# pingpongshow/RIA

Hardware: AMD Instinct MI355X
Metric: frames/s demod+LDPC-decoded, OFDM QAM16 R1/2 1024-FFT (higher is better)
Workload: dtype f32; 1 GPU; OFDM QAM16 R1/2 + LDPC min-sum, Watterson moderate fading 20 dB, 4400000 frames (100000 per step per GPU), full decodeFixedFrame; frame_samples=18432, batch_per_gpu=100000, channel=2

## Files before the change

### ria_amd/csrc/ldpc_fast.hip.h

```cpp
#pragma once
#include <hip/hip_runtime.h>
#include <stdint.h>

#include <type_traits>

#include "../../include/ria_gpu.h"
#include "devmath.h"
#include "ldpc_kernels.hip.h"

namespace ria {

struct ShapeR12 {
    static constexpr int NR = 6, NC = 6;
    static constexpr int kCascadeWaves = 3;
    static constexpr int kCv = 24;
    static constexpr int ne(int r) { constexpr int t[NR] = {6, 6, 5, 4, 2, 1}; return t[r]; }
    static constexpr int nm(int r) { constexpr int t[NR] = {6, 5, 4, 2, 1, 1}; return t[r]; }
    static constexpr int dv(int r) { constexpr int t[NC] = {5, 4, 4, 4, 4, 4}; return t[r]; }
};
struct ShapeR13 {
    static constexpr int NR = 6, NC = 6;
    static constexpr int kCascadeWaves = 3;
    static constexpr int kCv = 24;
    static constexpr int ne(int r) { constexpr int t[NR] = {6, 6, 5, 3, 3, 1}; return t[r]; }
// ... 108 lines not shown
}

template <int OFF>
__device__ __forceinline__ void lds_store_tid(uint32_t base, float v) {
    static_assert(OFF >= 0 && OFF < 65536, "16-bit DS offset");
    if constexpr (!kAddTid) {
        *(lds_float_ptr)(uintptr_t)(base + static_cast<uint32_t>(threadIdx.x) * 4u + OFF) = v;
        return;
    }
    asm volatile("s_mov_b32 m0, %1\n\ts_nop 0\n\tds_write_addtid_b32 %0 offset:%2" : : "v"(v), "s"(base), "n"(OFF) : "memory", "m0");
}
template <int N, int OFF, int STEP>
__device__ __forceinline__ void lds_store_tid_n(uint32_t base, const float (&v)[N]) {
    static_assert(N >= 1 && N <= 6 && OFF >= 0 && OFF + (N - 1) * STEP < 65536, "up to six 16-bit DS offsets");
    if constexpr (!kAddTid) {
#pragma unroll
        for (int i = 0; i < N; ++i) *(lds_float_ptr)(uintptr_t)(base + static_cast<uint32_t>(threadIdx.x) * 4u + OFF + i * STEP) = v[i];
        return;
    }
    if constexpr (N == 1)
        asm volatile("s_mov_b32 m0, %1\n\ts_nop 0\n\tds_write_addtid_b32 %0 offset:%2" : : "v"(v[0]), "s"(base), "n"(OFF) : "memory", "m0");
    else if constexpr (N == 2)
        asm volatile("s_mov_b32 m0, %2\n\ts_nop 0\n\tds_write_addtid_b32 %0 offset:%3\n\tds_write_addtid_b32 %1 offset:%4"
                     : : "v"(v[0]), "v"(v[1]), "s"(base), "n"(OFF), "n"(OFF + STEP) : "memory", "m0");
    else if constexpr (N == 3)
        asm volatile("s_mov_b32 m0, %3\n\ts_nop 0\n\tds_write_addtid_b32 %0 offset:%4\n\tds_write_addtid_b32 %1 offset:%5\n\tds_write_addtid_b32 %2 offset:%6"
                     : : "v"(v[0]), "v"(v[1]), "v"(v[2]), "s"(base), "n"(OFF), "n"(OFF + STEP), "n"(OFF + 2 * STEP) : "memory", "m0");
    else if constexpr (N == 4)
        asm volatile("s_mov_b32 m0, %4\n\ts_nop 0\n\tds_write_addtid_b32 %0 offset:%5\n\tds_write_addtid_b32 %1 offset:%6\n\tds_write_addtid_b32 %2 offset:%7\n\tds_write_addtid_b32 %3 offset:%8"
                     : : "v"(v[0]), "v"(v[1]), "v"(v[2]), "v"(v[3]), "s"(base), "n"(OFF), "n"(OFF + STEP), "n"(OFF + 2 * STEP), "n"(OFF + 3 * STEP) : "memory", "m0");
    else if constexpr (N == 5)
        asm volatile("s_mov_b32 m0, %5\n\ts_nop 0\n\tds_write_addtid_b32 %0 offset:%6\n\tds_write_addtid_b32 %1 offset:%7\n\tds_write_addtid_b32 %2 offset:%8\n\tds_write_addtid_b32 %3 offset:%9\n\tds_write_addtid_b32 %4 offset:%10"
                     : : "v"(v[0]), "v"(v[1]), "v"(v[2]), "v"(v[3]), "v"(v[4]), "s"(base), "n"(OFF), "n"(OFF + STEP), "n"(OFF + 2 * STEP), "n"(OFF + 3 * STEP), "n"(OFF + 4 * STEP) : "memory", "m0");
    else
        asm volatile("s_mov_b32 m0, %6\n\ts_nop 0\n\tds_write_addtid_b32 %0 offset:%7\n\tds_write_addtid_b32 %1 offset:%8\n\tds_write_addtid_b32 %2 offset:%9\n\tds_write_addtid_b32 %3 offset:%10\n\tds_write_addtid_b32 %4 offset:%11\n\tds_write_addtid_b32 %5 offset:%12"
                     : : "v"(v[0]), "v"(v[1]), "v"(v[2]), "v"(v[3]), "v"(v[4]), "v"(v[5]), "s"(base), "n"(OFF), "n"(OFF + STEP), "n"(OFF + 2 * STEP), "n"(OFF + 3 * STEP), "n"(OFF + 4 * STEP), "n"(OFF + 5 * STEP) : "memory", "m0");
}
__device__ __forceinline__ uint32_t med3u(uint32_t a, uint32_t b, uint32_t c) {
    uint32_t d;
    asm("v_med3_u32 %0, %1, %2, %3" : "=v"(d) : "v"(a), "v"(b), "v"(c));
    return d;
}
__device__ __forceinline__ float med3_abs(float x, float b, float c) { return __builtin_amdgcn_fmed3f(__builtin_fabsf(x), b, c); }
__device__ __forceinline__ float min_abs(float x, float b) { return __builtin_fminf(__builtin_fabsf(x), b); }
__device__ __forceinline__ float min3_abs(float a, float b, float c) { return __builtin_fminf(__builtin_fminf(__builtin_fabsf(a), __builtin_fabsf(b)), __builtin_fabsf(c)); }
__device__ __forceinline__ float med3_abs3(float a, float b, float c) { return __builtin_amdgcn_fmed3f(__builtin_fabsf(a), __builtin_fabsf(b), __builtin_fabsf(c)); }
__device__ __forceinline__ float min2_abs(float a, float b) { return __builtin_fminf(__builtin_fabsf(a), __builtin_fabsf(b)); }
__device__ __forceinline__ float max2_abs(float a, float b) { return __builtin_fmaxf(__builtin_fabsf(a), __builtin_fabsf(b)); }
__device__ __forceinline__ float min_raw(float a, float b) { return __builtin_fminf(a, b); }
template <int N>
__device__ __forceinline__ void two_smallest_abs(const float (&w)[N], float& lo, float& mid) {
    static_assert(N >= 2 && N <= 7, "row degree");
    if constexpr (N == 2) { lo = min2_abs(w[0], w[1]); mid = max2_abs(w[0], w[1]); }
    else {
        lo = min3_abs(w[0], w[1], w[2]); mid = med3_abs3(w[0], w[1], w[2]);
        if constexpr (N >= 6) {
            const float l2 = min3_abs(w[3], w[4], w[5]), m2 = med3_abs3(w[3], w[4], w[5]);
            const float x = min_raw(mid, m2);
            mid = __builtin_amdgcn_fmed3f(lo, l2, x);
            lo = min_raw(lo, l2);
            if constexpr (N == 7) { mid = med3_abs(w[6], lo, mid); lo = min_abs(w[6], lo); }
        } else {
            if constexpr (N >= 4) { mid = med3_abs(w[3], lo, mid); lo = min_abs(w[3], lo); }
            if constexpr (N >= 5) { mid = med3_abs(w[4], lo, mid); lo = min_abs(w[4], lo); }
        }
    }
}
__device__ __forceinline__ uint32_t bfi(uint32_t mask, uint32_t a, uint32_t b) { return (mask & a) | (~mask & b); }

__device__ __forceinline__ float llr_canon(float x) {
    x = (x < 1e30f) ? x : 1e30f;
    x = (-1e30f < x) ? x : -1e30f;
    return x + 0.0f;
}

#ifndef RIA_SINGLE_PREFETCH
#define RIA_SINGLE_PREFETCH 2
#endif
template <class S, int NCV = (kCvRegs ? 1024 : S::kCv), int PF = RIA_SINGLE_PREFETCH>
__device__ inline int fast_decode(FastState<S>& st, const FastCode& c, unsigned char* __restrict__ lds,
                                  float factor, int max_iter, int lane, bool* ok) {
    using I = ShapeInfo<S>;
    const uint32_t lane4 = lds_addr(lds) + static_cast<uint32_t>(lane) * 4u;
    const uint32_t kAbs = 0x7fffffffu;
    const uint32_t m0base = lds_addr(lds);
    static_for<0, S::NR>([&](auto R_) __attribute__((always_inline)) {
        constexpr int r = decltype(R_)::value;
#pragma unroll
        for (int s = 0; s < S::ne(r); ++s) {
            const float v0 = 0.0f;
            if (I::row_off(r) + s < NCV) st.cv[I::row_off(r) + s] = v0;
            else lds_sf(lane4 + 256u * (I::row_off(r) + s), v0);
        }
    });
#pragma unroll
    for (int r = 0; r < S::NC; ++r) lds_sf(lane4 + 4u * (I::tot_word + 64 * r), st.li[r]);
    lds_sf(lane4 + 4u * I::zero_word, 0.0f);
    lds_sf(lane4 + 4u * I::big_word, kPadTotal);
#pragma unroll
    for (int r = 0; r < S::NR; ++r) { st.pv[r] = st.lp[r]; st.pt[r] = 0.0f; }
    wave_sync();
    float hi = __builtin_inff();
    int it = 0;
    bool success = false;
    for (; it < max_iter; ++it) {
        uint32_t syn = 0;
        float tt[I::TS];
        auto gather_round = [&](auto G_) __attribute__((always_inline)) {
            constexpr int g = decltype(G_)::value;
            if constexpr (g < S::NR) {
#pragma unroll
                for (int s = 0; s < S::ne(g); ++s) tt[I::row_off(g) + s] = lds_f(st.rv[I::row_off(g) + s]);
            }
        };
        static_for<0, PF>([&](auto G_) __attribute__((always_inline)) { gather_round(G_); });
        static_for<0, S::NR>([&](auto R_) __attribute__((always_inline)) {
            constexpr int r = decltype(R_)::value;
            constexpr int NE = S::ne(r);
            constexpr int off = I::row_off(r);
            gather_round(std::integral_constant<int, r + PF>{});
            float t[NE], cold[NE];
#pragma unroll
            for (int s = 0; s < NE; ++s) {
                t[s] = tt[off + s];
                if (off + s < NCV) cold[s] = st.cv[off + s];
                else cold[s] = lds_f(lane4 + 256u * (off + s));
            }
            const float pvr = st.pv[r];
            uint32_t par = f2u(st.pt[r]);
            uint32_t sgn = f2u(pvr);
            float min1, min2;
            float v[NE + 1];
#pragma unroll
            for (int s = 0; s < NE; ++s) v[s] = t[s] - cold[s];
            v[NE] = pvr;
            two_smallest_abs<NE + 1>(v, min1, min2);
            min1 = min_raw(min1, hi);
            min2 = min_raw(min2, hi);
#pragma unroll
            for (int s = 0; s < NE; s += 2) {
                if (s + 1 < NE) {
                    par = __builtin_amdgcn_bitop3_b32(par, f2u(t[s]), f2u(t[s + 1]), 0x96);
                    sgn = __builtin_amdgcn_bitop3_b32(sgn, f2u(v[s]), f2u(v[s + 1]), 0x96);
                } else {
                    par ^= f2u(t[s]);
                    sgn ^= f2u(v[s]);
                }
            }
            syn |= par;
            const uint32_t dS = bfi(kAbs, f2u(min1) ^ f2u(min2), sgn);
            float o[NE];
#pragma unroll
            for (int s = 0; s < NE; ++s) o[s] = u2f(dS ^ f2u(__builtin_amdgcn_fmed3f(v[s], min2, -min2))) * factor;
            lds_store_tid_n<NE, 256 * off, 256>(m0base, o);
            static_for<0, NE>([&](auto S_) __attribute__((always_inline)) {
                constexpr int s = decltype(S_)::value;
                if constexpr (off + s < NCV) st.cv[off + s] = o[s];
            });
            {
                const float c2v = u2f(dS ^ f2u(__builtin_amdgcn_fmed3f(pvr, min2, -min2))) * factor;
                const float tot = st.lp[r] + c2v;
                st.pv[r] = tot - c2v;
                st.pt[r] = tot;
            }
        });
        if (it > 0 && __ballot(static_cast<int>(syn) < 0) == 0ull) { success = true; --it; break; }
        hi = 50.0f;
        wave_sync();
        constexpr int NCE = []() constexpr { int n = 0; for (int r = 0; r < S::NC; ++r) if (S::dv(r) > 0) n = r + 1; return n; }();
        float totv[NCE > 0 ? NCE : 1];
        static_for<0, NCE>([&](auto R_) __attribute__((always_inline)) {
            constexpr int r = decltype(R_)::value;
            constexpr int DV = S::dv(r);
            constexpr int off = I::col_off(r);
            float cv[DV > 0 ? DV : 1];
#pragma unroll
            for (int d = 0; d < DV; ++d) cv[d] = lds_f(st.cs[off + d]);
            float tot = st.li[r];
#pragma unroll
            for (int d = 0; d < DV; ++d) tot = tot + cv[d];
            totv[r] = tot;
        });
        static_for<0, (NCE + 5) / 6>([&](auto G_) __attribute__((always_inline)) {
            constexpr int g0 = 6 * decltype(G_)::value, gn = (NCE - g0 < 6) ? NCE - g0 : 6;
            float tv[gn];
#pragma unroll
            for (int i = 0; i < gn; ++i) tv[i] = totv[g0 + i];
            lds_store_tid_n<gn, 4 * (I::tot_word + 64 * g0), 256>(m0base, tv);
        });
        wave_sync();
    }
    if (!success) {
        uint32_t syn = 0;
        static_for<0, S::NR>([&](auto R_) __attribute__((always_inline)) {
            constexpr int r = decltype(R_)::value;
            constexpr int off = I::row_off(r);
            uint32_t par = f2u(st.pt[r]);
#pragma unroll
            for (int s = 0; s < S::ne(r); ++s) par ^= f2u(lds_f(st.rv[off + s]));
            syn |= par;
        });
        if (max_iter > 0 && __ballot(static_cast<int>(syn) < 0) == 0ull) { success = true; it = max_iter - 1; }
    }
    *ok = success;
    return success ? it : max_iter;
}

template <class S>
__device__ inline void fast_pack(const FastState<S>& st, const FastCode& c, unsigned char* lds, uint8_t* out, int nbytes,
                                 int lane) {
    using I = ShapeInfo<S>;
    (void)st;
    lane = opaque_lane(lane);
    unsigned long long* masks = reinterpret_cast<unsigned long long*>(lds);
    const int nr = (c.k + 63) / 64;
    for (int r = 0; r < nr; ++r) {
        const int j = lane + 64 * r;
        bool bit = false;
        if (j < c.k) bit = (f2u(lds_f(lds_addr(lds) + 4u * (I::tot_word + c.col_pos[j]))) >> 31) != 0u;
        unsigned long long mk = __ballot(bit);
        if (lane == 0) masks[r] = mk;
    }
    wave_sync();
    for (int b = lane; b < nbytes; b += 64) out[b] = static_cast<uint8_t>(__brev(static_cast<unsigned>(lds[b])) >> 24);
    wave_sync();
}

struct CascadeWin { unsigned int lock; unsigned int iters; uint8_t bytes[72]; };

struct DecodeCtl {
    unsigned int n_entries;
    unsigned int next_unit;
    unsigned int n_list1;
    unsigned int next_z;
    unsigned int queue_fault;
    unsigned int pad_[3];
};
#define RIA_QUEUE_GUARD(guard, total, ctl) \
    if (++(guard) > (total) + 2u) { if (threadIdx.x == 0) atomicExch(&(ctl)->queue_fault, 1u); break; }

constexpr int kNumFactors = 5;
__device__ __constant__ float kFactors[kNumFactors] = {0.9375f, 0.875f, 0.75f, 0.625f, 0.5f};
struct CwResult {
    uint8_t state[kNumFactors];
    uint8_t pad[kNumFactors - 2];
    uint16_t iters[kNumFactors];
};

struct FastDecodeArgs {
    FastCode c;
    const uint16_t* gather;
    const float* llr;
    int llr_stride;
    int n_frames;
    uint32_t flags;
    uint8_t* info_out;
    ria_decode_status* status;
    const uint16_t* crc_bit;
    const uint16_t* crc_init;
    DecodeCtl* ctl;
    unsigned int* entries;
    unsigned int* best;
    unsigned int* list1;
    CwResult* res;
    uint8_t* res_bytes;
    CascadeWin* win;
    float* staged;
    unsigned int* l1idx;
    unsigned int* l1hash;
    uint32_t* seed_ws;
};

constexpr int kStageFloats = 12 * 64;
constexpr int kStageFrameFloats = 2688;

constexpr float kIdleRowLlr = 1e30f;

template <class S>
__device__ inline void fast_gather_llr(FastState<S>& st, const FastCode& c, const float* fl, const uint16_t* gather,
                                       int cw, int lane) {
    lane = opaque_lane(lane);
#pragma unroll
    for (int r = 0; r < S::NC; ++r) {
        const uint32_t j = c.col_at[lane + 64 * r];
        st.li[r] = (j != 0xFFFFu) ? llr_canon(fl[gather[cw * 648 + j]]) : 0.0f;
    }
#pragma unroll
    for (int r = 0; r < S::NR; ++r) {
        const uint32_t i = c.check_at[lane + 64 * r];
        st.lp[r] = (i != 0xFFFFu) ? llr_canon(fl[gather[cw * 648 + c.k + i]]) : kIdleRowLlr;
    }
}

template <class S>
__device__ inline void fast_load_staged(FastState<S>& st, const float* __restrict__ src, int lane) {
    static_assert((S::NC + S::NR) * 64 <= kStageFloats, "stage slot too small");
    lane = opaque_lane(lane);
#pragma unroll
    for (int r = 0; r < S::NC; ++r) st.li[r] = src[r * 64 + lane];
#pragma unroll
    for (int r = 0; r < S::NR; ++r) st.lp[r] = src[(S::NC + r) * 64 + lane];
}

template <class S, int NCV = S::kCv>
__device__ inline void fast_unit(FastState<S>& st, const FastDecodeArgs& A, unsigned char* lds, unsigned fc, int f, int lane,
                                 const float* staged = nullptr) {
    const FastCode& c = A.c;
    if (staged) fast_load_staged(st, staged, lane);
    else fast_gather_llr(st, c, A.llr + static_cast<size_t>(fc >> 2) * A.llr_stride, A.gather, fc & 3, lane);
    bool ok;
    int it = fast_decode<S, NCV>(st, c, lds, kFactors[f], c.max_iter, lane, &ok);
    if (ok) fast_pack(st, c, lds, A.res_bytes + (static_cast<size_t>(fc) * kNumFactors + f) * c.bytes_per_cw,
                      c.bytes_per_cw, lane);
    if (lane == 0) { A.res[fc].state[f] = ok ? 2 : 1; A.res[fc].iters[f] = static_cast<uint16_t>(it); }
}

#ifndef RIA_PRIMARY_NCV
#define RIA_PRIMARY_NCV 0
#endif
template <class S>
__global__ __launch_bounds__(64) void fast_primary_kernel(FastDecodeArgs A) {
    extern __shared__ __attribute__((aligned(16))) unsigned char smem[];
    const int lane = threadIdx.x;
    const unsigned b = blockIdx.x, g = b >> 5, r = b & 31u, cw = r >> 3, x = r & 7u;
    const unsigned frame = 8u * g + x;
    if (frame >= static_cast<unsigned>(A.n_frames)) return;
    FastState<S> st;
    fast_load_tables(st, A.c, smem, lane);
    fast_unit<S, RIA_PRIMARY_NCV>(st, A, smem, 4u * frame + cw, 0, lane);
}

__global__ void fast_mark_kernel(FastDecodeArgs A) {
    int frame = blockIdx.x * blockDim.x + threadIdx.x;
    if (frame >= A.n_frames) return;
    if (!(A.flags & (RIA_DECODE_PHASE0 | RIA_DECODE_PERTURB))) return;
    bool failed = false;
    for (int cw = 0; cw < 4; ++cw) {
        unsigned fc = static_cast<unsigned>(frame) * 4u + cw;
        failed = failed || A.res[fc].state[0] != 2;
        if (failed) {
            const unsigned i = atomicAdd(&A.ctl->n_list1, 1u);
            A.list1[i] = fc;
            A.l1idx[fc] = i;
        }
    }
}

__device__ inline uint32_t fast_hash16(const float* fl, const uint16_t* gather, int cw, int lane) {
    const uint32_t mine = f2u(fl[gather[cw * 648 + (lane & 15)]]);
    uint32_t h = 0;
    for (int j = 0; j < 16; ++j) {
        uint32_t u = __shfl(mine, j);
        h ^= u + 0x9e3779b9u + (h << 6) + (h >> 2);
    }
    return h;
}

template <class S>
__global__ __launch_bounds__(256) void fast_stage_kernel(FastDecodeArgs A) {
    __shared__ float fr[kStageFrameFloats];
    const FastCode& c = A.c;
    const int tid = threadIdx.x, lane = tid & 63, wave = tid >> 6;
    const unsigned n = A.ctl->n_list1;
    const int nfl = A.llr_stride < kStageFrameFloats ? A.llr_stride : kStageFrameFloats;
    for (unsigned i = blockIdx.x; i < n; i += gridDim.x) {
        const unsigned fc = A.list1[i], cw = fc & 3u;
        const float* fl = A.llr + static_cast<size_t>(fc >> 2) * A.llr_stride;
        __syncthreads();
        for (int q = tid; q < nfl; q += 256) fr[q] = fl[q];
        __syncthreads();
        float* dst = A.staged + static_cast<size_t>(i) * kStageFloats;
        for (int r = wave; r < S::NC + S::NR; r += 4) {
            float v;
            if (r < S::NC) {
                const uint32_t j = c.col_at[lane + 64 * r];
                v = (j != 0xFFFFu) ? llr_canon(fr[A.gather[cw * 648 + j]]) : 0.0f;
            } else {
                const uint32_t k = c.check_at[lane + 64 * (r - S::NC)];
                v = (k != 0xFFFFu) ? llr_canon(fr[A.gather[cw * 648 + c.k + k]]) : kIdleRowLlr;
            }
            dst[r * 64 + lane] = v;
        }
        if (wave == 0) {
            const uint32_t h = fast_hash16(fr, A.gather, cw, lane);
            if (lane == 0) A.l1hash[i] = h;
        }
    }
}

template <class S>
__global__ __launch_bounds__(64) void fast_phase0_kernel(FastDecodeArgs A) {
    extern __shared__ __attribute__((aligned(16))) unsigned char smem[];
    const int lane = threadIdx.x;
    const unsigned total = A.ctl->n_list1 * 4u;
    if (blockIdx.x >= total) return;
    FastState<S> st;
    fast_load_tables(st, A.c, smem, lane);
    unsigned guard = 0;
    for (;;) {
        RIA_QUEUE_GUARD(guard, total, A.ctl)
        unsigned u = atomicAdd(&A.ctl->next_z, lane == 0 ? 1u : 0u);
        u = __builtin_amdgcn_readfirstlane(u);
        if (u >= total) break;
        fast_unit<S>(st, A, smem, A.list1[u >> 2], 1 + static_cast<int>(u & 3u), lane, A.staged + static_cast<size_t>(u >> 2) * kStageFloats);
    }
}

__global__ void fast_chain_kernel(FastDecodeArgs A) {
    int frame = blockIdx.x * blockDim.x + threadIdx.x;
    if (frame >= A.n_frames) return;
    const int bpc = A.c.bytes_per_cw;
    int f = 0;
    ria_decode_status* s = A.status + frame;
    for (int cw = 0; cw < 4; ++cw) {
        const unsigned fc = static_cast<unsigned>(frame) * 4u + cw;
        const CwResult r = A.res[fc];
        int accept = -1, attempts = 1, iters = r.iters[f];
        if (r.state[f] == 2) accept = f;
        else {
            if (A.flags & RIA_DECODE_PHASE0) {
                for (int t = 1; t <= 4 && accept < 0; ++t) { attempts++; if (r.state[t] == 2) { accept = t; iters = r.iters[t]; } }
                f = 0;
            }
            if (accept < 0 && (A.flags & RIA_DECODE_PERTURB)) {
                f = 1;
                unsigned e = atomicAdd(&A.ctl->n_entries, 1u);
                A.entries[e] = fc;
                A.best[e] = 0xFFFFFFFFu;
                A.win[e].lock = 0u;
            }
        }
        uint8_t* out = A.info_out + static_cast<size_t>(fc) * bpc;
        if (accept >= 0) {
            const uint8_t* src = A.res_bytes + (static_cast<size_t>(fc) * kNumFactors + accept) * bpc;
            for (int b = 0; b < bpc; ++b) out[b] = src[b];
        } else {
            for (int b = 0; b < bpc; ++b) out[b] = 0;
        }
        s->cw_ok[cw] = accept >= 0 ? 1 : 0;
        s->iterations[cw] = static_cast<uint16_t>(iters);
        s->attempts[cw] = static_cast<uint8_t>(attempts);
    }
}

#ifndef RIA_CASCADE_GROUP
#define RIA_CASCADE_GROUP 4
#endif
constexpr int kCascadeGroup = RIA_CASCADE_GROUP;
constexpr unsigned kCascadeGroups = (kRetryAttempts + kCascadeGroup - 1) / kCascadeGroup;
constexpr size_t kSeedWsWords = static_cast<size_t>(kCascadeGroup) * 624;

template <class S>
__device__ inline float fast_perturb(FastState<S>& st, const FastCode& c, const float* base_i, const float* base_p,
                                     uint32_t* mt, float* normal, const uint32_t* ws, int j, int a, int lane) {
    uint32_t seed; float sigma, factor; int kind;
    lane = opaque_lane(lane);
    retry_transform_params(a, 0u, &seed, &sigma, &factor, &kind);
    const bool noise = sigma != 0.0f;
    if (noise) {
        mt_load_group_state<kCascadeGroup>(mt, ws, j, lane);
        normal648_state(mt, normal, lane);
    }
    auto tf = [&](float v, float nz) {
        if (kind == 1) { v = (v < 10.0f) ? v : 10.0f; v = (-10.0f < v) ? v : -10.0f; }
        else if (kind == 2) v = v * 0.5f;
        else if (kind == 3) { v = (v < 6.0f) ? v : 6.0f; v = (-6.0f < v) ? v : -6.0f; }
        else if (kind == 4) v = (v >= 0.0f) ? 1.0f : -1.0f;
        else if (kind == 5) v = v * 0.25f;
        return v + (nz * sigma + 0.0f);
    };
#pragma unroll
    for (int r = 0; r < S::NC; ++r) {
        const uint32_t q = c.col_at[lane + 64 * r];
        const float nz = (noise && q != 0xFFFFu) ? normal[q] : 0.0f;
        st.li[r] = (q != 0xFFFFu) ? llr_canon(tf(base_i[r], nz)) : 0.0f;
    }
#pragma unroll
    for (int r = 0; r < S::NR; ++r) {
        const uint32_t i = c.check_at[lane + 64 * r];
        const float nz = (noise && i != 0xFFFFu) ? normal[c.k + i] : 0.0f;
        st.lp[r] = (i != 0xFFFFu) ? llr_canon(tf(base_p[r], nz)) : kIdleRowLlr;
    }
    wave_sync();
    return factor;
}

template <class S>
__global__ __launch_bounds__(64) __attribute__((amdgpu_waves_per_eu(S::kCascadeWaves))) void fast_cascade_kernel(FastDecodeArgs A) {
    extern __shared__ __attribute__((aligned(16))) unsigned char smem[];
    const FastCode& c = A.c;
    const int lane = threadIdx.x;
    float* msg = reinterpret_cast<float*>(smem);
    const unsigned int n_entries = A.ctl->n_entries;
    const unsigned int total = n_entries * kCascadeGroups;
    if (total == 0) return;
    FastState<S> st;
    fast_load_tables(st, c, smem, lane);
    unsigned guard = 0;
    for (;;) {
        RIA_QUEUE_GUARD(guard, total, A.ctl)
        unsigned int u = atomicAdd(&A.ctl->next_unit, lane == 0 ? 1u : 0u);
        u = __builtin_amdgcn_readfirstlane(u);
        if (u >= total) break;
        const unsigned int g = u / n_entries, e = u - g * n_entries, a0 = g * kCascadeGroup;
        unsigned int b = __hip_atomic_load(&A.best[e], __ATOMIC_RELAXED, __HIP_MEMORY_SCOPE_AGENT);
        b = __builtin_amdgcn_readfirstlane(b);
        if (b < a0) continue;
        const unsigned int li = A.l1idx[A.entries[e]];
        uint32_t* ws = A.seed_ws + static_cast<size_t>(blockIdx.x) * kSeedWsWords;
        mt_seed_group<kCascadeGroup>(ws, A.l1hash[li], a0, opaque_lane(lane));
#pragma unroll 1
        for (int j = 0; j < kCascadeGroup; ++j) {
            const unsigned int a = a0 + static_cast<unsigned>(j);
            if (a >= kRetryAttempts) break;
            if (j > 0) {
                b = __hip_atomic_load(&A.best[e], __ATOMIC_RELAXED, __HIP_MEMORY_SCOPE_AGENT);
                b = __builtin_amdgcn_readfirstlane(b);
                if (b < a) break;
            }
            fast_load_staged(st, A.staged + static_cast<size_t>(li) * kStageFloats, lane);
            float bi[S::NC], bp[S::NR];
#pragma unroll
            for (int r = 0; r < S::NC; ++r) bi[r] = st.li[r];
#pragma unroll
            for (int r = 0; r < S::NR; ++r) bp[r] = st.lp[r];
            float factor = fast_perturb(st, c, bi, bp, reinterpret_cast<uint32_t*>(msg), msg + 640, ws, j, static_cast<int>(a), lane);
            bool ok;
            const int it = fast_decode<S>(st, c, smem, factor, c.max_iter, lane, &ok);
            if (!ok) continue;
            unsigned int prev = atomicMin(&A.best[e], lane == 0 ? a : 0xFFFFFFFFu);
            prev = __builtin_amdgcn_readfirstlane(prev);
            if (a < prev) {
                CascadeWin* w = A.win + e;
                bool mine = false;
                for (unsigned spin = 0; spin < (1u << 20); ++spin) {
                    unsigned got = atomicCAS(&w->lock, 0u, lane == 0 ? 1u : 0u);
                    got = __builtin_amdgcn_readfirstlane(got);
                    if (got == 0u) { mine = true; break; }
                    __builtin_amdgcn_s_sleep(1);
                }
                if (!mine) { if (lane == 0) atomicExch(&A.ctl->queue_fault, 1u); break; }
                __threadfence();
                unsigned int cur = __hip_atomic_load(&A.best[e], __ATOMIC_RELAXED, __HIP_MEMORY_SCOPE_AGENT);
                cur = __builtin_amdgcn_readfirstlane(cur);
                if (cur == a) {
                    fast_pack(st, c, smem, w->bytes, c.bytes_per_cw, lane);
                    if (lane == 0) w->iters = static_cast<unsigned int>(it);
                }
                __threadfence();
                if (lane == 0) atomicExch(&w->lock, 0u);
            }
            break;
        }
    }
}

__global__ __launch_bounds__(256) void fast_finalize_kernel(FastDecodeArgs A) {
    const unsigned int n_entries = A.ctl->n_entries;
    const int bpc = A.c.bytes_per_cw;
    for (unsigned int e = blockIdx.x * blockDim.x + threadIdx.x; e < n_entries; e += gridDim.x * blockDim.x) {
        const unsigned int fc = A.entries[e], frame = fc >> 2, cw = fc & 3;
        const unsigned int a = A.best[e];
        ria_decode_status* s = A.status + frame;
        if (a >= 34u) { s->attempts[cw] = static_cast<uint8_t>(s->attempts[cw] + 34); continue; }
        const CascadeWin* w = A.win + e;
        uint8_t* out = A.info_out + (static_cast<size_t>(frame) * 4 + cw) * bpc;
        for (int b = 0; b < bpc; ++b) out[b] = w->bytes[b];
        s->cw_ok[cw] = 1;
        s->iterations[cw] = static_cast<uint16_t>(w->iters);
        s->attempts[cw] = static_cast<uint8_t>(s->attempts[cw] + a + 1);
    }
}

__device__ inline bool decode_fault_mark(const DecodeCtl* ctl, ria_decode_status* s, uint8_t* info, int info_bytes, int lane) {
    if (__hip_atomic_load(&ctl->queue_fault, __ATOMIC_RELAXED, __HIP_MEMORY_SCOPE_AGENT) == 0u) return false;
    for (int b = lane; b < info_bytes; b += 64) info[b] = 0;
    if (lane == 0) {
        for (int cw = 0; cw < 4; ++cw) s->cw_ok[cw] = 0;
        s->frame_valid = 0; s->needs_recovery = 0; s->reserved[0] = 0; s->reserved[1] = 0xEE;
    }
    return true;
}
constexpr uint8_t kDecodeFaultMarker = 0xEE;

__global__ __launch_bounds__(256) void frame_validate_kernel(uint8_t* __restrict__ info, int bpc, int n_frames,
                                                             const uint16_t* __restrict__ crc_bit,
                                                             const uint16_t* __restrict__ crc_init,
                                                             ria_decode_status* __restrict__ status, const DecodeCtl* ctl) {
    __shared__ uint8_t flat_all[4][4 * 68];
    const int lane = threadIdx.x & 63, wave = threadIdx.x >> 6;
    const int frame = blockIdx.x * 4 + wave;
    if (frame >= n_frames) return;
    uint8_t* flat = flat_all[wave];
    ria_decode_status* s = status + frame;
    if (decode_fault_mark(ctl, s, info + static_cast<size_t>(frame) * 4 * bpc, 4 * bpc, lane)) return;
    const bool all_ok = s->cw_ok[0] && s->cw_ok[1] && s->cw_ok[2] && s->cw_ok[3];
    int valid = 0, quirk = 0;
    if (all_ok) {
        for (int b = lane; b < 4 * bpc; b += 64) flat[b] = info[static_cast<size_t>(frame) * 4 * bpc + b];
        wave_sync();
        bool magic = flat[0] == 0x55 && flat[1] == 0x4C;
        int t = flat[2];
        bool ctl = (t == 0x10 || t == 0x11 || t == 0x16 || t == 0x17 || t == 0x20 || t == 0x21 || t == 0x15 || t == 0x40);
        int plen = (flat[13] << 8) | flat[14];
        int expected = ctl ? 20 : 17 + plen + 2;
        for (int cw = 1; cw < 4; ++cw) if (cw * bpc < expected && flat[cw * bpc] == 0xD5) quirk = 1;
        if (magic && !quirk) {
            if (ctl) {
                uint32_t crc = crc16_wave(flat, 18, crc_bit, crc_init, lane);
                valid = crc == static_cast<uint32_t>((flat[18] << 8) | flat[19]);
            } else {
                uint32_t hc = crc16_wave(flat, 15, crc_bit, crc_init, lane);
                if (hc == static_cast<uint32_t>((flat[15] << 8) | flat[16]) && expected <= 4 * bpc) {
                    uint32_t fc = crc16_wave(flat, expected - 2, crc_bit, crc_init, lane);
                    valid = fc == static_cast<uint32_t>((flat[expected - 2] << 8) | flat[expected - 1]);
                }
            }
        }
    }
    if (lane == 0) {
        s->frame_valid = static_cast<uint8_t>(valid);
        s->needs_recovery = static_cast<uint8_t>(all_ok && !valid);
        s->reserved[0] = static_cast<uint8_t>(quirk);
        s->reserved[1] = 0;
    }
}

__global__ __launch_bounds__(256) void decode_fault_kernel(const DecodeCtl* ctl, ria_decode_status* __restrict__ status, uint8_t* __restrict__ info,
                                                           int bpc, int n_frames) {
    const int lane = threadIdx.x & 63, frame = blockIdx.x * 4 + (threadIdx.x >> 6);
    if (frame >= n_frames) return;
    (void)decode_fault_mark(ctl, status + frame, info + static_cast<size_t>(frame) * 4 * bpc, 4 * bpc, lane);
}

#ifndef RIA_ROWS_NCV
#define RIA_ROWS_NCV (kCvRegs ? 1024 : S::kCv)
#endif
#ifdef RIA_ROWS_WAVES
#define RIA_ROWS_ATTR __attribute__((amdgpu_waves_per_eu(RIA_ROWS_WAVES, RIA_ROWS_WAVES)))
#else
#define RIA_ROWS_ATTR
#endif
template <class S>
__global__ __launch_bounds__(64) RIA_ROWS_ATTR void fast_rows_kernel(FastCode c, const float* __restrict__ llr, int n_cw, int max_iter,
                                                       float factor, uint8_t* __restrict__ out, uint8_t* __restrict__ ok_out,
                                                       uint16_t* __restrict__ iters_out) {
    extern __shared__ __attribute__((aligned(16))) unsigned char smem[];
    const int lane = threadIdx.x;
    FastState<S> st;
    fast_load_tables(st, c, smem, lane);
    const int nb = (c.k + 7) / 8;
    for (int cw = blockIdx.x; cw < n_cw; cw += gridDim.x) {
        const float* l = llr + static_cast<size_t>(cw) * 648;
        const int ln = opaque_lane(lane);
#pragma unroll
        for (int r = 0; r < S::NC; ++r) { const uint32_t j = c.col_at[ln + 64 * r]; st.li[r] = (j != 0xFFFFu) ? llr_canon(l[j]) : 0.0f; }
#pragma unroll
        for (int r = 0; r < S::NR; ++r) { const uint32_t i = c.check_at[ln + 64 * r]; st.lp[r] = (i != 0xFFFFu) ? llr_canon(l[c.k + i]) : kIdleRowLlr; }
        bool ok;
        int it = fast_decode<S, RIA_ROWS_NCV>(st, c, smem, factor, max_iter, lane, &ok);
        fast_pack(st, c, smem, out + static_cast<size_t>(cw) * nb, nb, lane);
        if (lane == 0) { ok_out[cw] = ok ? 1 : 0; iters_out[cw] = static_cast<uint16_t>(it); }
    }
}

template <class S>
__global__ __launch_bounds__(64) void fast_robust_kernel(FastCode c, const float* __restrict__ llr, int n_cw,
                                                         uint8_t* __restrict__ out, uint8_t* __restrict__ ok_out,
                                                         uint16_t* __restrict__ iters_out, uint8_t* __restrict__ tries_out) {
    extern __shared__ __attribute__((aligned(16))) unsigned char smem[];
    const int lane = threadIdx.x;
    FastState<S> st;
    fast_load_tables(st, c, smem, lane);
    const int nb = (c.k + 7) / 8;
    for (int cw = blockIdx.x; cw < n_cw; cw += gridDim.x) {
        const float* l = llr + static_cast<size_t>(cw) * 648;
#pragma unroll
        for (int r = 0; r < S::NC; ++r) { const uint32_t j = c.col_at[lane + 64 * r]; st.li[r] = (j != 0xFFFFu) ? llr_canon(l[j]) : 0.0f; }
#pragma unroll
        for (int r = 0; r < S::NR; ++r) { const uint32_t i = c.check_at[lane + 64 * r]; st.lp[r] = (i != 0xFFFFu) ? llr_canon(l[c.k + i]) : kIdleRowLlr; }
        bool ok = false;
        int it = 0, tries = 0;
#pragma unroll 1
        for (int f = 0; f < kNumFactors && !ok; ++f) {
            it = fast_decode(st, c, smem, kFactors[f], c.max_iter, lane, &ok);
            ++tries;
        }
        fast_pack(st, c, smem, out + static_cast<size_t>(cw) * nb, nb, lane);
        if (lane == 0) {
            ok_out[cw] = ok ? 1 : 0; iters_out[cw] = static_cast<uint16_t>(it);
            if (tries_out) tries_out[cw] = static_cast<uint8_t>(tries);
        }
    }
}

}
```

### ria_amd/csrc/recovery_kernels.hip.h

```cpp
#pragma once
#include <hip/hip_runtime.h>
#include <stdint.h>

#include "ldpc_fast.hip.h"
#include "sort_exact.hpp"

namespace ria {

struct RecCtx {
    uint8_t* cw;
    uint8_t* fd;
    uint8_t* trial;
    Suspect* sus;
    int* stack;
    uint16_t* sd;
    uint16_t* lists;
    int sus_cap;
    unsigned long long* dbg;
    int bpc;
    const uint16_t* crc_bit;
    const uint16_t* crc_init;
    int lane;
};

// ... 149 lines not shown
    if (lane < fin) mine = v[lane];
    int rank = 0;
    for (int j = 0; j < fin; ++j) {
        const float kj = __builtin_bit_cast(float, __builtin_amdgcn_readlane(__builtin_bit_cast(int, mine.abs_llr), j));
        rank += (kj < mine.abs_llr || (j < lane && !(mine.abs_llr < kj))) ? 1 : 0;
    }
    wave_sync();
    if (lane < fin) v[rank] = mine;
    wave_sync();
}

constexpr int kRecOverflow = 2;
constexpr int kRecSmallCap = 320;
template <class LlrFn>
__device__ inline int rec_search(const RecCtx& x, LlrFn llr) {
    const int bpc = x.bpc, lane = x.lane;
    auto stamp = [&](int k) { if (x.dbg && lane == 0) x.dbg[k] = __builtin_readcyclecounter(); };
    stamp(0);
    const int flen = rec_reassemble(x, x.fd);
    if (flen == 0) {
        const int tb = bpc * 8;
        const uint8_t* c0 = x.cw;
        const uint32_t hsyn = crc16_wave(c0, 15, x.crc_bit, x.crc_init, lane) ^ static_cast<uint32_t>((c0[15] << 8) | c0[16]);
        const uint32_t msyn = static_cast<uint32_t>((c0[0] << 8) | c0[1]) ^ 0x554Cu;
        auto dh = [&](int b) -> uint32_t {
            const int by = b >> 3, bit = b & 7;
            if (by < 15) return x.crc_bit[(14 - by) * 8 + bit];
            if (by == 15) return 1u << (8 + bit);
            if (by == 16) return 1u << bit;
            return 0u;
        };
        auto dm = [&](int b) -> uint32_t {
            const int by = b >> 3, bit = b & 7;
            if (by == 0) return 1u << (8 + bit);
            if (by == 1) return 1u << bit;
            return 0u;
        };
        const uint32_t d0 = (dh(lane) << 16) | dm(lane), d1 = (dh(lane + 64) << 16) | dm(lane + 64), d2 = (dh(lane + 128) << 16) | dm(lane + 128);
        const uint32_t syn2 = (hsyn << 16) | msyn;
        auto d_of = [&](int b) -> uint32_t {
            if (b >= 192) return 0u;
            const uint32_t r = (b < 64) ? d0 : (b < 128) ? d1 : d2;
            return static_cast<uint32_t>(__builtin_amdgcn_readlane(static_cast<int>(r), b & 63));
        };
        auto for_matches = [&](uint32_t want, int from, auto f) -> bool {
            for (int base = 0; base < 192 && base < tb; base += 64) {
                const int b = base + lane;
                const uint32_t dv = (base == 0) ? d0 : (base == 64) ? d1 : d2;
                unsigned long long hits = __ballot(b >= from && b < tb && dv == want);
                while (hits) {
                    const int bb = base + __builtin_ctzll(hits);
                    hits &= hits - 1;
                    if (f(bb)) return true;
                }
            }
            if (want == 0u)
                for (int bb = (from > 192 ? from : 192); bb < tb; ++bb) if (f(bb)) return true;
            return false;
        };
        if (for_matches(syn2, 0, [&](int bb) {
                rec_flip(x, bb >> 3, bb & 7);
                if (rec_try(x)) return true;
                rec_flip(x, bb >> 3, bb & 7);
                return false; })) return true;
        for (int b1 = 0; b1 < tb; ++b1) {
            const uint32_t want = syn2 ^ d_of(b1);
            if (want == 0u) {
                rec_flip(x, b1 >> 3, b1 & 7);
                const int tl = rec_reassemble(x, x.trial);
                bool ctl2 = false; int plen2 = 0;
                const bool hdr = tl > 0 && rec_parse_header(x, x.trial, tl, &ctl2, &plen2);
                const int exp2 = 17 + plen2 + 2;
                bool done = false;
                if (hdr && !ctl2 && tl >= exp2) {
                    const uint32_t s2 = static_cast<uint32_t>((x.trial[exp2 - 2] << 8) | x.trial[exp2 - 1]) ^
                                        crc16_wave(x.trial, exp2 - 2, x.crc_bit, x.crc_init, lane);
                    const int from = (b1 + 1 > 136) ? b1 + 1 : 136;
                    for (int base = (from & ~63); base < tb && !done; base += 64) {
                        const int b2 = base + lane, by = b2 >> 3, bit = b2 & 7;
                        uint32_t dl = 0u;
                        if (b2 < tb) {
                            if (by < exp2 - 2) dl = x.crc_bit[(exp2 - 3 - by) * 8 + bit];
                            else if (by < exp2) dl = 1u << (bit + 8 * (exp2 - 1 - by));
                        }
                        unsigned long long hits = __ballot(b2 >= from && b2 < tb && dl == s2);
                        while (hits && !done) {
                            const int bb = base + __builtin_ctzll(hits);
                            hits &= hits - 1;
                            rec_flip(x, bb >> 3, bb & 7);
                            if (rec_try(x)) done = true; else rec_flip(x, bb >> 3, bb & 7);
                        }
                    }
                } else if (hdr && ctl2) {
                    done = true;
                } else if (!hdr) {
                    for (int bb = (b1 + 1 > 136) ? b1 + 1 : 136; bb < tb && !done; ++bb) {
                        rec_flip(x, bb >> 3, bb & 7);
                        if (rec_try(x)) done = true; else rec_flip(x, bb >> 3, bb & 7);
                    }
                }
                if (done) return true;
                rec_flip(x, b1 >> 3, b1 & 7);
                continue;
            }
            if (for_matches(want, b1 + 1, [&](int bb) {
                    rec_flip(x, b1 >> 3, b1 & 7);
                    rec_flip(x, bb >> 3, bb & 7);
                    if (rec_try(x)) return true;
                    rec_flip(x, bb >> 3, bb & 7);
                    rec_flip(x, b1 >> 3, b1 & 7);
                    return false; })) return true;
        }
        return false;
    }
    bool ctl; int plen;
    if (!rec_parse_header(x, x.fd, flen, &ctl, &plen) || ctl) return false;
    const int expected = 17 + plen + 2;
    if (flen < expected) return false;
    const uint32_t stored = static_cast<uint32_t>((x.fd[expected - 2] << 8) | x.fd[expected - 1]);
    const int data_bytes = expected - 2, data_bits = data_bytes * 8;
    const uint32_t syn = stored ^ crc16_wave(x.fd, data_bytes, x.crc_bit, x.crc_init, lane);
    auto delta = [&](int p) -> uint32_t { return x.crc_bit[(data_bytes - 1 - (p >> 3)) * 8 + (p & 7)]; };
    auto fix = [&](int p) {
        const int fb = p >> 3, c = fb / bpc;
        if (c < 4) rec_flip(x, c * 68 + fb % bpc, p & 7);
    };
    {
        constexpr int kMaxRounds = (4 * 68 * 8 + 63) / 64;
        uint32_t dl[kMaxRounds];
#pragma unroll
        for (int q = 0; q < kMaxRounds; ++q) { const int p = 64 * q + lane; dl[q] = (p < data_bits) ? delta(p) : 0xFFFFFFFFu; }
#pragma unroll
        for (int q = 0; q < kMaxRounds; ++q) {
            const int base = 64 * q, p = base + lane;
            if (base >= data_bits) break;
            unsigned long long hits = __ballot(p < data_bits && dl[q] == syn && (p >> 3) / bpc < 4);
            if (hits) { fix(base + __builtin_ctzll(hits)); return true; }
        }
    }
    for (int bit = 0; bit < 16; ++bit)
        if (syn == (1u << bit)) {
            const int fb = (bit >= 8) ? expected - 2 : expected - 1, c = fb / bpc;
            if (c < 4) { rec_flip(x, c * 68 + fb % bpc, bit & 7); return true; }
        }
    stamp(1);
    int ns_all = 0;
    const int cw_bits = (bpc * 8 < 648) ? bpc * 8 : 648;
    for (int c = 0; c < 4; ++c) {
        constexpr int kMaxRounds = 9;
        float lv[kMaxRounds];
#pragma unroll
        for (int q = 0; q < kMaxRounds; ++q) {
            const int i = 64 * q + lane;
            lv[q] = (i < cw_bits && ((c * bpc * 8 + i) >> 3) < data_bytes) ? llr(c, i) : 0.0f;
        }
#pragma unroll
        for (int q = 0; q < kMaxRounds; ++q) {
            const int base = 64 * q;
            if (base >= cw_bits) break;
            const int i = base + lane;
            bool is = false;
            const float l = lv[q];
            int fbit = 0;
            if (i < cw_bits) {
                fbit = c * bpc * 8 + i;
                if ((fbit >> 3) < data_bytes) {
                    const int chb = (l < 0.0f) ? 1 : 0, db = (x.cw[c * 68 + (i >> 3)] >> (i & 7)) & 1;
                    is = chb != db;
                }
            }
            const unsigned long long mk = __ballot(is);
            if (is) {
                const int at = ns_all + __popcll(mk & ((1ull << lane) - 1ull));
                if (at < x.sus_cap) {
                    x.sus[at].frame_bit = fbit;
                    x.sus[at].abs_llr = fabs_(l);
                }
            }
            ns_all += __popcll(mk);
        }
    }
    if (ns_all > x.sus_cap) return kRecOverflow;
    wave_sync();
    stamp(2);
    rec_sort_suspects_wave(x, ns_all, 30);
    stamp(3);
    if (x.dbg && lane == 0) x.dbg[7] = static_cast<unsigned long long>(ns_all);
    const int ns = ns_all < 30 ? ns_all : 30;
    const uint32_t my = (lane < ns) ? delta(x.sus[lane].frame_bit) : 0u;
    auto sd_at = [&](int a) -> uint32_t { return static_cast<uint32_t>(__builtin_amdgcn_readlane(static_cast<int>(my), a)); };
    auto sd_lane = [&](int a) -> uint32_t { return static_cast<uint32_t>(__shfl(static_cast<int>(my), a)); };
    auto sd_at_lane = [&](uint32_t mine, int p, int ln) -> uint32_t { (void)p; (void)ln; return mine; };
    auto attempt = [&](int n_idx, int a, int b, int c, int d) -> bool {
        const int idx[4] = {a, b, c, d};
        for (int q = 0; q < n_idx; ++q) fix(x.sus[idx[q]].frame_bit);
        if (rec_try(x)) return true;
        for (int q = 0; q < n_idx; ++q) fix(x.sus[idx[q]].frame_bit);
        return false;
    };
    auto try_class = [&](int n_idx, int n_members, int n_prefixes, auto prefix_of) -> bool {
        for (int base = 0; base < n_prefixes; base += 64) {
            const bool valid = base + lane < n_prefixes;
            const int p = valid ? base + lane : n_prefixes - 1;
            int ia = 0, ib = 0, ic = 0;
            uint32_t want = 0u;
            int last_from = n_members;
            prefix_of(p, ia, ib, ic, want, last_from);
            uint32_t found = 0u;
            for (int d = 1; d < n_members; ++d) {
                const uint32_t sdv = sd_at(d);
                if (valid && d >= last_from && sdv == want) found |= 1u << d;
            }
            unsigned long long lanes = __ballot(found != 0u);
            while (lanes) {
                const int l = __builtin_ctzll(lanes);
                lanes &= lanes - 1;
                uint32_t f = static_cast<uint32_t>(__builtin_amdgcn_readlane(static_cast<int>(found), l));
                const int pa = __builtin_amdgcn_readlane(ia, l), pb = __builtin_amdgcn_readlane(ib, l), pc = __builtin_amdgcn_readlane(ic, l);
                while (f) {
                    const int d = __builtin_ctz(f);
                    f &= f - 1;
                    const bool ok = (n_idx == 2) ? attempt(2, pa, d, 0, 0) : (n_idx == 3) ? attempt(3, pa, pb, d, 0) : attempt(4, pa, pb, pc, d);
                    if (ok) return true;
                }
            }
        }
        return false;
    };
    if (try_class(2, ns, ns, [&](int p, int& ia, int& ib, int& ic, uint32_t& want, int& from) {
            (void)ib; (void)ic; ia = p; want = syn ^ sd_at_lane(my, p, lane); from = p + 1; })) return true;
    stamp(4);
    {
        const int np = ns * (ns - 1) / 2;
        if (try_class(3, ns, np, [&](int p, int& ia, int& ib, int& ic, uint32_t& want, int& from) {
                (void)ic;
                int a = 0, rem = p;
                while (rem >= ns - 1 - a) { rem -= ns - 1 - a; ++a; }
                ia = a; ib = a + 1 + rem;
                want = syn ^ sd_lane(ia) ^ sd_lane(ib); from = ib + 1; })) return true;
    }
    {
        const int n4 = ns < 15 ? ns : 15;
        const int np = n4 * (n4 - 1) * (n4 - 2) / 6;
        if (try_class(4, n4, np, [&](int p, int& ia, int& ib, int& ic, uint32_t& want, int& from) {
                int a = 0, rem = p;
                for (;;) { const int m = n4 - 1 - a, cnt = m * (m - 1) / 2; if (rem < cnt) break; rem -= cnt; ++a; }
                int b = a + 1;
                for (;;) { const int cnt = n4 - 1 - b; if (rem < cnt) break; rem -= cnt; ++b; }
                ia = a; ib = b; ic = b + 1 + rem;
                want = syn ^ sd_lane(ia) ^ sd_lane(ib) ^ sd_lane(ic); from = ic + 1; })) return true;
    }
    return false;
}

struct RecoveryArgs {
    FastDecodeArgs d;
    unsigned int* n_flagged;
    unsigned int* flagged;
    unsigned int* n_list2;
    unsigned int* list2;
    unsigned int* n_stage2;
    unsigned int* stage2;
    unsigned int* next_fill;
    unsigned long long* dbg;
    unsigned int* n_overflow;
    unsigned int* overflow;
    int list_units_now;
    uint8_t* info_c;
    float* rows_c;
    uint8_t* redec_ok;
    uint8_t* redec_bytes;
};

__global__ void recovery_list_kernel(RecoveryArgs R) {
    int frame = blockIdx.x * blockDim.x + threadIdx.x;
    if (frame >= R.d.n_frames || !R.d.status[frame].needs_recovery) return;
    R.flagged[atomicAdd(R.n_flagged, 1u)] = static_cast<unsigned>(frame);
    if (!R.list_units_now) return;
    for (int cw = 0; cw < 4; ++cw) {
        unsigned fc = static_cast<unsigned>(frame) * 4u + cw, mask = 0;
        for (int f = 1; f <= 4; ++f)
            if (R.d.res[fc].state[f] == 0) mask |= 1u << (f - 1);
        if (mask) R.list2[atomicAdd(R.n_list2, 1u)] = (fc << 4) | mask;
    }
}
template <class S>
__global__ __launch_bounds__(64) void recovery_fill_kernel(RecoveryArgs R) {
    extern __shared__ __attribute__((aligned(16))) unsigned char smem[];
    const unsigned total = *R.n_list2 * 4u;
    if (blockIdx.x >= total) return;
    FastState<S> st;
    fast_load_tables(st, R.d.c, smem, threadIdx.x);
    unsigned guard = 0;
    for (;;) {
        RIA_QUEUE_GUARD(guard, total, R.d.ctl)
        unsigned u = atomicAdd(R.next_fill, threadIdx.x == 0 ? 1u : 0u);
        u = __builtin_amdgcn_readfirstlane(u);
        if (u >= total) break;
        const unsigned e = R.list2[u >> 2], fc = e >> 4;
        const int f = 1 + static_cast<int>(u & 3u);
        if (!((e >> (f - 1)) & 1u)) continue;
        const FastCode& c = R.d.c;
        const int lane = threadIdx.x;
        fast_gather_llr(st, c, R.d.llr + static_cast<size_t>(fc >> 2) * R.d.llr_stride, R.d.gather, fc & 3, lane);
        bool ok;
        const int it = fast_decode<S>(st, c, smem, kFactors[f], c.max_iter, lane, &ok);
        if (ok) fast_pack(st, c, smem, R.d.res_bytes + (static_cast<size_t>(fc) * kNumFactors + f) * c.bytes_per_cw, c.bytes_per_cw, lane);
        if (lane == 0) { R.d.res[fc].state[f] = ok ? 2 : 1; R.d.res[fc].iters[f] = static_cast<uint16_t>(it); }
    }
}
__global__ __launch_bounds__(256) void recovery_gather_kernel(RecoveryArgs R) {
    const unsigned q = blockIdx.x;
    if (q >= *R.n_flagged) return;
    const unsigned frame = R.flagged[q];
    const int bpc = R.d.c.bytes_per_cw, ib = 4 * bpc;
    for (int i = threadIdx.x; i < ib; i += 256) R.info_c[static_cast<size_t>(q) * ib + i] = R.d.info_out[static_cast<size_t>(frame) * ib + i];
    const float* fl = R.d.llr + static_cast<size_t>(frame) * R.d.llr_stride;
    for (int i = threadIdx.x; i < 4 * 648; i += 256) R.rows_c[static_cast<size_t>(q) * 4 * 648 + i] = fl[R.d.gather[i]];
    const int forder[4] = {2, 3, 4, 1};
    if (threadIdx.x < 16) {
        int at = threadIdx.x >> 2, cw = threadIdx.x & 3;
        R.redec_ok[static_cast<size_t>(q) * 16 + threadIdx.x] = R.d.res[frame * 4u + cw].state[forder[at]] == 2 ? 1 : 0;
    }
    for (int i = threadIdx.x; i < 16 * bpc; i += 256) {
        int slot = i / bpc, b = i - slot * bpc, at = slot >> 2, cw = slot & 3;
        R.redec_bytes[static_cast<size_t>(q) * 16 * bpc + i] =
            R.d.res_bytes[(static_cast<size_t>(frame * 4u + cw) * kNumFactors + forder[at]) * bpc + b];
    }
}


__host__ __device__ inline int recovery_sus_cap(int bpc, bool big) { return big ? 4 * bpc * 8 : (kRecSmallCap < 4 * bpc * 8 ? kRecSmallCap : 4 * bpc * 8); }
__host__ __device__ inline int recovery_lds_bytes(int bpc, bool big = true) {
    const int cap = recovery_sus_cap(bpc, big);
    return 1024 + cap * 8 + 192 * 4 + 2 * (cap / 2 + 32) * 2 + 64;
}

__device__ inline void rec_setup(RecCtx& x, unsigned char* smem, const RecoveryArgs& R, int lane, bool big = true) {
    x.sus_cap = recovery_sus_cap(R.d.c.bytes_per_cw, big);
    x.cw = smem; x.fd = smem + 272; x.trial = smem + 544;
    x.sd = reinterpret_cast<uint16_t*>(smem + 816);
    x.stack = reinterpret_cast<int*>(smem + 1024);
    x.sus = reinterpret_cast<Suspect*>(smem + 1024 + 192 * 4);
    x.lists = reinterpret_cast<uint16_t*>(smem + 1024 + 192 * 4 + x.sus_cap * 8);
    x.bpc = R.d.c.bytes_per_cw; x.crc_bit = R.d.crc_bit; x.crc_init = R.d.crc_init; x.lane = lane;
    x.dbg = nullptr;
}
__device__ inline void rec_load_cw(const RecCtx& x, const uint8_t* info, int lane) {
    for (int i = lane; i < 4 * 68; i += 64) { const int c = i / 68, b = i - c * 68; x.cw[i] = (b < x.bpc) ? info[c * x.bpc + b] : 0; }
    wave_sync();
}
__device__ inline void rec_publish(const RecCtx& x, const RecoveryArgs& R, unsigned frame, uint8_t* info, bool good, int lane) {
    wave_sync();
    for (int i = lane; i < 4 * x.bpc; i += 64) { const int c = i / x.bpc, b = i - c * x.bpc; info[i] = good ? x.cw[c * 68 + b] : 0; }
    if (lane == 0) {
        ria_decode_status* s = R.d.status + frame;
        s->needs_recovery = 0;
        s->frame_valid = good ? 1 : 0;
        for (int c = 0; c < 4; ++c) s->cw_ok[c] = good ? 1 : 0;
    }
}

__global__ __launch_bounds__(64) void recovery_stage1_kernel(RecoveryArgs R) {
    extern __shared__ __attribute__((aligned(16))) unsigned char smem[];
    const unsigned q = blockIdx.x;
    if (q >= *R.n_flagged) return;
    const unsigned frame = R.flagged[q];
    const int lane = threadIdx.x;
    RecCtx x;
    rec_setup(x, smem, R, lane, true);
    if (R.dbg) x.dbg = R.dbg + static_cast<size_t>(frame) * 8;
    uint8_t* info = R.d.info_out + static_cast<size_t>(frame) * 4 * x.bpc;
    rec_load_cw(x, info, lane);
    const float* fl = R.d.llr + static_cast<size_t>(frame) * R.d.llr_stride;
    const uint16_t* gather = R.d.gather;
    const int good = rec_search(x, [&](int c, int i) { return fl[gather[c * 648 + i]]; });
    if (x.dbg && lane == 0) { x.dbg[6] = __builtin_readcyclecounter(); x.dbg[5] = static_cast<unsigned long long>(good); }
    if (good == kRecOverflow) return;
    if (good) { rec_publish(x, R, frame, info, true, lane); return; }
    const unsigned fc = frame * 4u + static_cast<unsigned>((lane >> 2) & 3);
    const int f = 1 + (lane & 3);
    const bool need = lane < 16 && R.d.res[fc].state[f] == 0;
    const unsigned long long mk = __ballot(need);
    const unsigned mine = static_cast<unsigned>(mk >> (lane & 12)) & 15u;
    const bool writer = lane < 16 && (lane & 3) == 0 && mine != 0u;
    const unsigned long long wk = __ballot(writer);
    unsigned base = 0;
    if (lane == 0) {
        R.stage2[atomicAdd(R.n_stage2, 1u)] = frame;
        if (wk) base = atomicAdd(R.n_list2, static_cast<unsigned>(__popcll(wk)));
    }
    base = static_cast<unsigned>(__builtin_amdgcn_readfirstlane(static_cast<int>(base)));
    if (writer) R.list2[base + __popcll(wk & ((1ull << lane) - 1ull))] = (fc << 4) | mine;
}

__global__ __launch_bounds__(64) void recovery_stage2_kernel(RecoveryArgs R) {
    extern __shared__ __attribute__((aligned(16))) unsigned char smem[];
    const unsigned q = blockIdx.x;
    if (q >= *R.n_stage2) return;
    const unsigned frame = R.stage2[q];
    const int lane = threadIdx.x;
    RecCtx x;
    rec_setup(x, smem, R, lane);
    const int bpc = x.bpc;
    uint8_t* info = R.d.info_out + static_cast<size_t>(frame) * 4 * bpc;
    rec_load_cw(x, info, lane);
    bool good = false;
    const int forder[4] = {2, 3, 4, 1};
    for (int at = 0; at < 4 && !good; ++at)
        for (int c = 0; c < 4 && !good; ++c) {
            const unsigned fc = frame * 4u + c;
            if (R.d.res[fc].state[forder[at]] != 2) continue;
            const uint8_t* rd = R.d.res_bytes + (static_cast<size_t>(fc) * kNumFactors + forder[at]) * bpc;
            bool diff = false;
            for (int b = lane; b < bpc; b += 64) diff = diff || rd[b] != x.cw[c * 68 + b];
            if (__ballot(diff) == 0ull) continue;
            uint8_t keep0 = 0, keep1 = 0;
            wave_sync();
            if (lane < bpc) { keep0 = x.cw[c * 68 + lane]; x.cw[c * 68 + lane] = rd[lane]; }
            if (lane + 64 < bpc) { keep1 = x.cw[c * 68 + lane + 64]; x.cw[c * 68 + lane + 64] = rd[lane + 64]; }
            wave_sync();
            if (rec_try(x)) { good = true; break; }
            if (lane < bpc) x.cw[c * 68 + lane] = keep0;
            if (lane + 64 < bpc) x.cw[c * 68 + lane + 64] = keep1;
            wave_sync();
        }
    rec_publish(x, R, frame, info, good, lane);
}

}
```

Before: 1.535 million frames/s.

## Order phase0 work factor-major and skip later factors once an earlier succeeds

The phase0 retry queue now walks all listed codewords for factor 1 first, then factor 2, and so on. Before each unit it atomically checks whether any earlier factor has already converged for that codeword and skips the decode if so, which avoids redundant min-sum decodes that the chain kernel would never use. Results are published with an agent-scope atomic store so other workgroups can see them. The recovery fill kernel also reuses the staged canonical LLRs through l1idx instead of re-gathering from global memory, and the mark kernel now sets a sentinel for unlisted codewords. The skip depends on timing, so which attempts run is nondeterministic, and the chain kernel has to handle factors left unset.

New measurement: 1.556 million frames/s (median of 6 runs). 1.4% higher.

```diff
diff --git a/ria_amd/csrc/ldpc_fast.hip.h b/ria_amd/csrc/ldpc_fast.hip.h
--- a/ria_amd/csrc/ldpc_fast.hip.h
+++ b/ria_amd/csrc/ldpc_fast.hip.h
@@ -434,6 +434,13 @@
     for (int r = 0; r < S::NR; ++r) st.lp[r] = src[(S::NC + r) * 64 + lane];
 }
 
+__device__ inline void fast_publish(CwResult* res, unsigned fc, int f, bool ok, int it, int lane) {
+    if (lane == 0) {
+        res[fc].iters[f] = static_cast<uint16_t>(it);
+        __hip_atomic_store(&res[fc].state[f], static_cast<uint8_t>(ok ? 2 : 1), __ATOMIC_RELAXED, __HIP_MEMORY_SCOPE_AGENT);
+    }
+}
+
 template <class S, int NCV = S::kCv>
 __device__ inline void fast_unit(FastState<S>& st, const FastDecodeArgs& A, unsigned char* lds, unsigned fc, int f, int lane,
                                  const float* staged = nullptr) {
@@ -444,7 +451,7 @@
     int it = fast_decode<S, NCV>(st, c, lds, kFactors[f], c.max_iter, lane, &ok);
     if (ok) fast_pack(st, c, lds, A.res_bytes + (static_cast<size_t>(fc) * kNumFactors + f) * c.bytes_per_cw,
                       c.bytes_per_cw, lane);
-    if (lane == 0) { A.res[fc].state[f] = ok ? 2 : 1; A.res[fc].iters[f] = static_cast<uint16_t>(it); }
+    fast_publish(A.res, fc, f, ok, it, lane);
 }
 
 #ifndef RIA_PRIMARY_NCV
@@ -461,6 +468,8 @@
     fast_load_tables(st, A.c, smem, lane);
     fast_unit<S, RIA_PRIMARY_NCV>(st, A, smem, 4u * frame + cw, 0, lane);
 }
+
+constexpr unsigned int kNotListed = 0xFFFFFFFFu;
 
 __global__ void fast_mark_kernel(FastDecodeArgs A) {
     int frame = blockIdx.x * blockDim.x + threadIdx.x;
@@ -474,6 +483,8 @@
             const unsigned i = atomicAdd(&A.ctl->n_list1, 1u);
             A.list1[i] = fc;
             A.l1idx[fc] = i;
+        } else {
+            A.l1idx[fc] = kNotListed;
         }
     }
 }
@@ -520,11 +531,14 @@
     }
 }
 
+#ifndef RIA_EAGER_FACTORS
+#define RIA_EAGER_FACTORS 0
+#endif
 template <class S>
 __global__ __launch_bounds__(64) void fast_phase0_kernel(FastDecodeArgs A) {
     extern __shared__ __attribute__((aligned(16))) unsigned char smem[];
     const int lane = threadIdx.x;
-    const unsigned total = A.ctl->n_list1 * 4u;
+    const unsigned n_list1 = A.ctl->n_list1, total = n_list1 * 4u;
     if (blockIdx.x >= total) return;
     FastState<S> st;
     fast_load_tables(st, A.c, smem, lane);
@@ -534,7 +548,22 @@
         unsigned u = atomicAdd(&A.ctl->next_z, lane == 0 ? 1u : 0u);
         u = __builtin_amdgcn_readfirstlane(u);
         if (u >= total) break;
-        fast_unit<S>(st, A, smem, A.list1[u >> 2], 1 + static_cast<int>(u & 3u), lane, A.staged + static_cast<size_t>(u >> 2) * kStageFloats);
+#if RIA_EAGER_FACTORS
+        const unsigned entry = u >> 2;
+        const int t = 1 + static_cast<int>(u & 3u);
+        const unsigned fc = A.list1[entry];
+#else
+        const unsigned tq = u / n_list1, entry = u - tq * n_list1;
+        const int t = 1 + static_cast<int>(tq);
+        const unsigned fc = A.list1[entry];
+        bool done = false;
+        for (int k = 1; k < t; ++k) {
+            const unsigned sk = __hip_atomic_load(&A.res[fc].state[k], __ATOMIC_RELAXED, __HIP_MEMORY_SCOPE_AGENT);
+            done = done || __builtin_amdgcn_readfirstlane(sk) == 2u;
+        }
+        if (done) continue;
+#endif
+        fast_unit<S>(st, A, smem, fc, t, lane, A.staged + static_cast<size_t>(entry) * kStageFloats);
     }
 }
 
diff --git a/ria_amd/csrc/recovery_kernels.hip.h b/ria_amd/csrc/recovery_kernels.hip.h
--- a/ria_amd/csrc/recovery_kernels.hip.h
+++ b/ria_amd/csrc/recovery_kernels.hip.h
@@ -475,11 +475,14 @@
         if (!((e >> (f - 1)) & 1u)) continue;
         const FastCode& c = R.d.c;
         const int lane = threadIdx.x;
-        fast_gather_llr(st, c, R.d.llr + static_cast<size_t>(fc >> 2) * R.d.llr_stride, R.d.gather, fc & 3, lane);
+        unsigned li = kNotListed;
+        if (R.d.flags & (RIA_DECODE_PHASE0 | RIA_DECODE_PERTURB)) li = static_cast<unsigned>(__builtin_amdgcn_readfirstlane(static_cast<int>(R.d.l1idx[fc])));
+        if (li != kNotListed) fast_load_staged(st, R.d.staged + static_cast<size_t>(li) * kStageFloats, lane);
+        else fast_gather_llr(st, c, R.d.llr + static_cast<size_t>(fc >> 2) * R.d.llr_stride, R.d.gather, fc & 3, lane);
         bool ok;
         const int it = fast_decode<S>(st, c, smem, kFactors[f], c.max_iter, lane, &ok);
         if (ok) fast_pack(st, c, smem, R.d.res_bytes + (static_cast<size_t>(fc) * kNumFactors + f) * c.bytes_per_cw, c.bytes_per_cw, lane);
-        if (lane == 0) { R.d.res[fc].state[f] = ok ? 2 : 1; R.d.res[fc].iters[f] = static_cast<uint16_t>(it); }
+        fast_publish(R.d.res, fc, f, ok, it, lane);
     }
 }
 __global__ __launch_bounds__(256) void recovery_gather_kernel(RecoveryArgs R) {
```
